# ShittyWizard/DiplomJourney

Measured on AMD Instinct MI355X. Metric: candidate N-step rollouts/sec + MPC-step p50 latency, 1/2/4/8 MI355X, higher is better.
Workload: dtype f64

## Files before the change

### diplomjourney_amd/csrc/mpc_episode.h

```cpp
#pragma once

#include <hip/hip_runtime.h>
#include <stddef.h>
#include <stdint.h>

#include "../../include/mpc_rollout.h"
#include "mpc_device.h"
#include "mpc_winner.h"

namespace mpc {

struct EpisodeHead {
  Consts K;
  double incumbent;
  double x, y, phi, v, beta;
  double x_t, y_t, x_0, y_0;
  double t;
  uint64_t seed;
  int64_t step;
  int32_t p, m, steps_for_slowing, episodes;
  int32_t nv, nb;
  int32_t recursive;
  int32_t has_traj;
};
// ... 26 lines not shown
constexpr int kStagedWords = kStoredWords + kEarlyWords;
static_assert(kStagedWords <= 64, "staged head: one word per lane");
constexpr int kLogWords = static_cast<int>(sizeof(mpc_episode_log_t) / 8);
static_assert(sizeof(EpisodeHead) % 8 == 0 && kHeadWords <= 64, "head: one word per lane");
static_assert(sizeof(mpc_episode_log_t) % 8 == 0 && kLogWords <= 64, "log: one word per lane");

__device__ __forceinline__ mpc_episode_log_t* log_slot(mpc_episode_log_t* log, int cap,
                                                       int64_t step) {
  return (log && cap > 0) ? &log[step % cap] : nullptr;
}

__device__ __forceinline__ bool early_pose_ok(const mpc_episode_config_t& c, const EpisodeHead& H,
                                              double x, double y) {
  if (c.stop_rule == 1 && x == H.x && y == H.y && H.recursive >= 1) return false;
  const double ex = H.x_t - x, ey = H.y_t - y;
  return !(ex * ex + ey * ey <= c.eps);
}

constexpr int kEpMaxGrid = 64;

constexpr int kConstsWords = static_cast<int>(sizeof(Consts) / 4);
constexpr int kPubWords = kConstsWords + 2;
static_assert(sizeof(Consts) % 4 == 0 && kPubWords <= 64, "published words: one wave");

struct EpisodeState {
  EpisodeHead h;
  StaleTraj st;
  EarlyPub early;
  double grid_v[kEpMaxGrid];
  double grid_b[kEpMaxGrid];
  uint32_t done;
  uint32_t chain_error;
  uint32_t p2p_seq;
  alignas(128) uint64_t chain_pub[kPubWords];
  alignas(128) uint64_t gathered_tag;
};
static_assert(offsetof(EpisodeState, st) == sizeof(EpisodeHead), "stale trajectory follows the head");
static_assert(offsetof(EpisodeState, early) == kStoredWords * 8, "EarlyPub follows the stale trajectory");

__device__ inline Consts episode_consts(const EpisodeHead& S, double x, double y, double phi,
                                        double L, double t_a, double t_b) {
  mpc_problem_t p;
  p.x = x;
  p.y = y;
  p.phi = phi;
  p.x_t = S.x_t;
  p.y_t = S.y_t;
  p.x_0 = S.x_0;
  p.y_0 = S.y_0;
  p.L = L;
  p.t_a = t_a;
  p.t_b = t_b;
  return consts_from_problem(p);
}

__device__ inline void episode_restart(const mpc_episode_config_t& c, EpisodeHead& S) {
  S.x = c.start_x;
  S.y = c.start_y;
  S.phi = c.start_phi;
// ... 40 lines not shown
                      !(c.max_steps > 0 && S.p + 1 > c.max_steps);
  const int k = S.m == 2 ? 2 : (S.m == 1 ? 1 : 0);
  E.k = common ? k : -1;
  E.x = S.has_traj ? st.ot[k][0] : S.x;
  E.y = S.has_traj ? st.ot[k][1] : S.y;
  E.ph = S.has_traj ? st.ot[k][2] : S.phi;
  E.alt = early_pose_ok(c, S, E.x, E.y) ? 1 : 0;
}

__global__ void k_episode_reset(mpc_episode_config_t c, EpisodeState* __restrict__ S) {
  if (threadIdx.x != 0) return;
  EpisodeHead H = {};
  episode_restart(c, H);
  episode_prepare(c, H);
  EarlyPub E;
  episode_early_prepare(c, H, S->st, E);
  S->early = E;
  S->h = H;
  S->done = 0u;
  S->chain_error = 0u;
  S->p2p_seq = 0u;
  for (int q = 0; q < kPubWords; ++q) S->chain_pub[q] = 0ull;
  S->gathered_tag = 0ull;
}

__device__ inline void turn_target(double ax, double ay, double aphi, double d, double R,
                                   double sign, double& tx, double& ty) {
  const double pi = 3.141592653589793;
  double sn, cs;
  if (pi / 2 <= aphi && aphi <= 3 * pi / 2) {
    if (aphi <= pi) {
      trig::sincos_fast(aphi - pi / 2, &sn, &cs);
      tx = ax - sign * d * cs - R * sn;
      ty = ay - sign * d * sn + R * cs;
    } else {
      trig::sincos_fast(aphi - pi, &sn, &cs);
      tx = ax + sign * d * sn - R * cs;
      ty = ay - sign * d * cs - R * sn;
    }
  } else if (aphi <= 2 * pi) {
    trig::sincos_fast(aphi - 3 * pi / 2, &sn, &cs);
    tx = ax + sign * d * cs + R * sn;
    ty = ay + sign * d * sn - R * cs;
  } else {
    trig::sincos_fast(aphi, &sn, &cs);
    tx = ax - sign * d * sn + R * cs;
// ... 137 lines not shown
```

### diplomjourney_amd/csrc/mpc_finalize.h

```cpp
#pragma once

#include <hip/hip_runtime.h>
#include <stddef.h>
#include <stdint.h>

#include <type_traits>

#include "../../include/mpc_rollout.h"
#include "mpc_argmin.h"
#include "mpc_device.h"
#include "mpc_episode.h"
#include "mpc_lanes.h"
#include "mpc_winner.h"

namespace mpc {

__device__ __forceinline__ void store_update(EpisodeHead* H, const uint64_t* s_head,
                                             mpc_episode_log_t* slot, const uint64_t* s_log,
                                             uint64_t* chain_pub, int chain_words,
                                             uint32_t epoch = 0, bool published = false,
                                             const uint32_t* pub = nullptr) {
  const int q = threadIdx.x;
  if (chain_pub && q < chain_words && !published) {
    if (epoch) {
// ... 39 lines not shown
  base = reinterpret_cast<const Rec*>(
      (static_cast<uint64_t>(static_cast<uint32_t>(__builtin_amdgcn_readfirstlane(
           static_cast<int>(ab >> 32)))) << 32) |
      static_cast<uint32_t>(__builtin_amdgcn_readfirstlane(static_cast<int>(ab))));
  asm volatile(
      "s_nop 4\n\t"
      "global_load_dwordx4 %0, %8, %16 sc1\n\t"
      "global_load_dwordx4 %1, %9, %16 sc1\n\t"
      "global_load_dwordx4 %2, %10, %16 sc1\n\t"
      "global_load_dwordx4 %3, %11, %16 sc1\n\t"
      "global_load_dwordx4 %4, %12, %16 sc1\n\t"
      "global_load_dwordx4 %5, %13, %16 sc1\n\t"
      "global_load_dwordx4 %6, %14, %16 sc1\n\t"
      "global_load_dwordx4 %7, %15, %16 sc1\n\t"
      "s_waitcnt vmcnt(0)"
      : "=&v"(r[0]), "=&v"(r[1]), "=&v"(r[2]), "=&v"(r[3]), "=&v"(r[4]), "=&v"(r[5]),
        "=&v"(r[6]), "=&v"(r[7])
      : "v"(o[0]), "v"(o[1]), "v"(o[2]), "v"(o[3]), "v"(o[4]), "v"(o[5]), "v"(o[6]), "v"(o[7]),
        "s"(base)
      : "memory");
}

struct NoRecSrc {};
template <int INTEG, int ROT, bool KDEV, int NT, bool SC1, bool GEN = false, bool TILED = false,
          class Src = NoRecSrc>
__device__ __forceinline__ void finalize_block(
    const Rec* __restrict__ part, int n_part, const Consts& K, const double* __restrict__ v,
    const double* __restrict__ b, int64_t n_cand, int n_steps, int64_t index_base,
    double incumbent, mpc_result_t* __restrict__ out, const mpc_episode_config_t& ecfg,
    const EpisodeHook& hook, EmitLds* lds, const Src& src = Src{}) {
  static_assert(NT >= 128, "head staging by wave 1");
  static_assert(MPC_MAX_STEPS * 3 <= NT, "trajectory stored one value per lane");
  __shared__ uint64_t s_head[kStagedWords];
  __shared__ mpc_episode_log_t s_log;
  __shared__ mpc_episode_log_t* s_slot;
  __shared__ uint64_t s_key[NT / 64];
  __shared__ int64_t s_idx[NT / 64];
  constexpr int kKWords = static_cast<int>(sizeof(Consts) / 4);
  __shared__ __attribute__((aligned(8))) uint32_t s_pub[64];
  __shared__ double2 s_sc[3];
  __shared__ int s_early, s_pose, s_sc_ready;
  uint64_t k = ~0ull;
  int64_t i = INT64_MAX;
  const bool stage = KDEV && hook.H && threadIdx.x >= 64 && threadIdx.x < 64 + kStagedWords;
  const uint64_t head_word =
      stage ? reinterpret_cast<const uint64_t*>(hook.H)[threadIdx.x - 64] : 0ull;
  if constexpr (!std::is_same_v<Src, NoRecSrc>) {
    src(k, i);
  } else if constexpr (SC1) {
    static_assert(kMaxBlocks <= 8 * NT, "load8_rec_sc1 covers 8 records per thread");
    const Rec* ptr[8];
    u64x2 r[8];
#pragma unroll
// ... 155 lines not shown
              if (pose == 1 && sc == 1) {
                Kp.s0 = s_sc[jj_w].x;
                Kp.c0 = s_sc[jj_w].y;
                pub = 1;
              }
            }
          }
          s_early = pub;
        }
        __builtin_amdgcn_fence(__ATOMIC_RELEASE, "wavefront");
        __builtin_amdgcn_wave_barrier();
        __builtin_amdgcn_fence(__ATOMIC_ACQUIRE, "wavefront");
        const int w3 = q - 192;
        if (s_early && w3 < hook.chain_pub_words)
          __hip_atomic_store(&hook.chain_pub[w3],
                             (static_cast<uint64_t>(s_pub[w3]) << 32) | hook.publish_epoch,
                             __ATOMIC_RELAXED, __HIP_MEMORY_SCOPE_AGENT);
      }
    };
    emit_winner<INTEG, ROT>(K, v, b, n_cand, n_steps, k, i, index_base + i, incumbent, out, lds,
                            &w, s_pv, s_pb, KDEV && hook.H, side_a, side_b, on_layer);
  }
  if (KDEV && hook.H) {
    const bool early = hook.publish_epoch && s_early;
    if (threadIdx.x == 0) {
      bool bad = false;
      episode_hook(ecfg, hook, w, *reinterpret_cast<EpisodeHead*>(s_head),
                   *reinterpret_cast<StaleTraj*>(&s_head[kHeadWords]), s_log, s_slot,
                   early ? s_pub : nullptr, &bad);
      if (bad && hook.chain_error) *hook.chain_error = 6u;
    }
    __syncthreads();
    if (hook.publish_epoch && threadIdx.x == 64) {
      EarlyPub E;
      episode_early_prepare(ecfg, *reinterpret_cast<const EpisodeHead*>(s_head),
                            *reinterpret_cast<const StaleTraj*>(&s_head[kHeadWords]), E);
      *reinterpret_cast<EarlyPub*>(reinterpret_cast<uint64_t*>(hook.H) + kStoredWords) = E;
    }
    store_update(hook.H, s_head, s_slot, reinterpret_cast<const uint64_t*>(&s_log),
                 hook.chain_pub, hook.chain_pub_words, hook.publish_epoch, early, s_pub);
    emit_winner_tail<INTEG, ROT>(K, n_steps, lds, out);
  }
}

template <int INTEG, int ROT>
__global__ __launch_bounds__(kFinBlock) void k_finalize_gen(
    const Rec* __restrict__ part, int n_part, const Consts* __restrict__ Kdev,
    const double* __restrict__ part_v, const double* __restrict__ part_b, int n_steps,
    int64_t index_base, const double* __restrict__ incumbent_dev,
    mpc_result_t* __restrict__ out, mpc_episode_config_t ecfg, EpisodeHook hook) {
  const Consts K = *Kdev;
  __shared__ EmitLds lds;
  finalize_block<INTEG, ROT, true, kFinBlock, false, true>(part, n_part, K, part_v, part_b, 0,
                                                           n_steps, index_base, *incumbent_dev,
                                                           out, ecfg, hook, &lds);
}

template <int INTEG, int ROT, bool KDEV, bool TILED = false>
__global__ __launch_bounds__(kFinBlock) void k_finalize(
    const Rec* __restrict__ part, int n_part, Consts Karg, const Consts* __restrict__ Kdev,
    const double* __restrict__ v, const double* __restrict__ b, int64_t n_cand, int n_steps,
    int64_t index_base, double incumbent_arg, const double* __restrict__ incumbent_dev,
    mpc_result_t* __restrict__ out, mpc_episode_config_t ecfg, EpisodeHook hook) {
  const Consts K = KDEV ? *Kdev : Karg;
// ... 54 lines not shown
```

### diplomjourney_amd/csrc/mpc_generated.h

```cpp
#pragma once

#include <hip/hip_runtime.h>
#include <stdint.h>

#include "mpc_argmin.h"
#include "mpc_device.h"
#include "mpc_episode.h"
#include "mpc_sampler.h"

namespace mpc {

__device__ inline void episode_grids(const mpc_episode_config_t& c, const EpisodeHead& S,
                                     double* s_v, double* s_b, int& nv_out, int& nb_out) {
  const int lane = threadIdx.x & 63;
  const uint64_t below = (lane == 0) ? 0ull : (~0ull >> (64 - lane));
  const int n_v = 1 + 2 * static_cast<int>(c.ratio_v);
  int nv = 0;
  double vmin = __builtin_inf();
  for (int base = 0; base < n_v; base += 64) {
    const int i = base + lane;
    const double cand = S.v + c.delta_v * (static_cast<double>(i) - c.ratio_v);
    const bool ok = i < n_v && !(cand < 0.0) && cand < c.v_max;
    const uint64_t m = __ballot(ok);
    const int pos = nv + __popcll(m & below);
    if (ok && pos < kEpMaxGrid) s_v[pos] = cand;
    if (S.steps_for_slowing > 0) {
      double mn = ok ? cand : __builtin_inf();
      for (int off = 32; off > 0; off >>= 1) mn = fmin(mn, __shfl_xor(mn, off, 64));
      vmin = fmin(vmin, mn);
    }
    nv += __popcll(m);
  }
  nv = nv < kEpMaxGrid ? nv : kEpMaxGrid;
  if (S.steps_for_slowing > 0 && nv > 0) {
    const double vel = vmin > c.v_min ? vmin : c.v_min;
// ... 177 lines not shown
```

### diplomjourney_amd/csrc/mpc_rollout.hip

```cpp
#include <hip/hip_ext.h>
#include <hip/hip_runtime.h>

#include <math.h>
#include <stdint.h>
#include <string.h>

#include <algorithm>
#include <mutex>
#include <type_traits>

#include "../../include/mpc_rollout.h"
#include "mpc_argmin.h"
#include "mpc_chain.h"
#include "mpc_comm.h"
#include "mpc_device.h"
#include "mpc_episode.h"
#include "mpc_episode_obs.h"
#include "mpc_episodes.h"
#include "mpc_exchange.h"
#include "mpc_finalize.h"
#include "mpc_ftepisodes.h"
#include "mpc_fulltree.h"
#include "mpc_generated.h"
#include "mpc_host_consts.h"
#include "mpc_kernels.h"
#include "mpc_lanes.h"
#include "mpc_run.h"
#include "mpc_sampler.h"
#include "mpc_winner.h"

namespace mpc {
namespace {

inline bool aligned16(const void* p) { return (reinterpret_cast<uintptr_t>(p) & 15u) == 0; }

inline int64_t cdiv(int64_t a, int64_t b) { return (a + b - 1) / b; }
// ... 652 lines not shown
            launched = hipFuncSetAttribute(
                           reinterpret_cast<const void*>(&k_rollout_generated<I, R, PL2>),
                           hipFuncAttributeMaxDynamicSharedMemorySize,
                           static_cast<int>(lds)) == hipSuccess;
          if (launched) {
            k_rollout_generated<I, R, PL2><<<grid, kBlock, lds, st>>>(
                *cfg, S, n_cand, n_steps, index_base, part, part_v, part_b);
            launched = hipPeekAtLastError() == hipSuccess;
          }
        },
        length_pow2(cfg->L));
    if (launched)
      k_finalize_gen<I, R><<<1, kFinBlock, 0, st>>>(part, static_cast<int>(grid), &S->h.K, part_v,
                                                    part_b, n_steps, index_base, &S->h.incumbent,
                                                    out, *cfg, hook);
  });
  if (!launched) {
    (void)hipGetLastError();
    return MPC_ERR_HIP;
  }
  return last_hip_status();
}

int mpc_episode_partials(void* state, const double* v_sc, const double* beta_sc, int64_t n_cand,
                         int32_t n_steps, int32_t integrator, void* ws, size_t ws_bytes,
                         mpc_stream_t stream) {
  if (check_episode_arrays(state, v_sc, beta_sc, n_cand, n_steps) != MPC_OK) return MPC_ERR_ARG;
  if (mode_ok(integrator) != MPC_OK) return MPC_ERR_UNSUPPORTED;
  if (!workspace_ok(ws, ws_bytes, n_cand, n_steps)) return MPC_ERR_WORKSPACE;
  EpisodeState* S = static_cast<EpisodeState*>(state);
  launch_rollout<true>(reinterpret_cast<hipStream_t>(stream), integrator, Consts{}, &S->h.K, v_sc,
                       beta_sc, n_cand, n_steps, static_cast<Rec*>(ws));
  return last_hip_status();
}

int mpc_episode_finalize(void* state, const double* v_sc, const double* beta_sc, int64_t n_cand,
                         int32_t n_steps, int64_t index_base, int32_t integrator, void* ws,
                         size_t ws_bytes, mpc_result_t* out, const mpc_episode_config_t* advance,
                         mpc_episode_log_t* log, int32_t log_capacity, mpc_stream_t stream) {
  const int a = check_episode_finish(state, v_sc, beta_sc, n_cand, n_steps, index_base, integrator,
                                     true, ws, ws_bytes, out, advance, log_capacity);
  if (a != MPC_OK) return a;
  EpisodeState* S = static_cast<EpisodeState*>(state);
  const int n_part = static_cast<int>(is_tiled(integrator)
                                          ? rollout_grid<kCplWide>(n_cand)
                                          : partial_count(v_sc, beta_sc, n_cand, false));
// ... 802 lines not shown
```

### diplomjourney_amd/device_episode.py

```python
import ctypes
import weakref

import torch

from . import native
from .abi import (CANDIDATE_BYTES, INTEGRATORS, IPC_HANDLE_BYTES, LOG_BYTES, MPC_LAYOUT_TILED,
                  MPC_MAX_OBSTACLES, MPC_TILE, RESULT_BYTES, MpcEpisodeLog, make_obstacles)
from .distributed import gather_bytes, gather_into, gather_results, reduce_int, shard_range
from .episode_config import ChainError, reference_episode_config
from .streams import _check_overlap_stream


def _is_tiled(controls):
    return isinstance(controls, torch.Tensor)


def _stop(events):
    if events:
        events[1].record()


class _ChainForm:
    pends_controls = False

# ... 4 lines not shown
class _OneGpuChain(_ChainForm):
    pends_controls = True

    def launch(self, ep, ctl, pend, events):
        vp, bp, integ = ep._ptrs(ctl)
        ws, ws_prev = ep._ws
        args = (1, ep._next_epoch(), vp, bp, *ep._shard, integ, ws.data_ptr(),
                ws_prev.data_ptr(), ws.numel(), *ep._prev_ptrs(pend), ep.local.data_ptr(), None, 0)
        if ep._n_obs or ep._obstacle_entries:
            log, cap, st = ep._tail()
            ep._C.mpc_episode_chain_step_obstacles(*ep._head, *ep._circles(), *args, log, cap,
                                                   ep._blocked_ptr(), st)
        else:
            ep._C.mpc_episode_chain_step(*ep._head, *args, *ep._tail())
        _stop(events)
        return ctl

    def flush(self, ep, pend):
        vp, bp, integ = ep._ptrs(pend)
        ws = ep._ws[1]
        ep._C.mpc_episode_finalize(
            ep.state.data_ptr(), vp, bp, *ep._shard, integ, ws.data_ptr(), ws.numel(),
            ep.local.data_ptr(), ctypes.byref(ep.cfg), *ep._tail())


class _P2PChain(_ChainForm):
    pends_controls = True

    def __init__(self, mailbox):
        self.mailbox = mailbox
        self.prev_epoch = 0

    def launch(self, ep, ctl, pend, events):
        vp, bp, integ = ep._ptrs(ctl)
        ws, ws_prev = ep._ws
        epoch = ep._next_epoch()
        ep._C.mpc_episode_p2p_step(
            *ep._head, epoch, self.prev_epoch if pend is not None else 0, vp, bp,
            *ep._shard, integ, ws.data_ptr(), ws_prev.data_ptr(), ws.numel(),
            *ep._prev_ptrs(pend), ctypes.c_void_p(self.mailbox.ptr), ep.world,
            ep.winner.data_ptr(), *ep._tail())
        _stop(events)
        self.prev_epoch = epoch
        return ctl

    def flush(self, ep, pend):
# ... 162 lines not shown
            raise ValueError(self._OBSTACLE_FORMS)
        self.cand = torch.zeros(CANDIDATE_BYTES, dtype=torch.uint8, device=dev)
        self.overlap = bool(overlap)
        if self.overlap and not (self.exchange and self.chain):
            raise ValueError("overlap: the chained exchange step only (exchange=True, chain=True)")
        if self.overlap and self.world > 32:
            raise ValueError("overlap: at most 32 ranks (gathered candidates staged in LDS)")
        self.p2p = bool(p2p)
        if self.p2p and (self.overlap or not (self.exchange and self.chain)):
            raise ValueError("p2p: the chained exchange step (exchange=True, chain=True), "
                             "not overlapped")
        self._mailbox = None
        self.p2p_status = None
        if self.p2p:
            self._p2p_setup(dev, bool(mailbox_uncached))
        self._form = (_OneGpuChain() if not self.exchange else
                      _P2PChain(self._mailbox) if self.p2p else
                      _OverlappedChain(self.world, dev) if self.overlap else _GatheredChain())
        if self.generate and self.exchange:
            raise ValueError("generated controls: one GPU (no exchange step)")
        self._gen_ws = None
        self._run_ws = None
        self._pending = None
        self._epoch = 0
        self._checked = {}
        self.steps_enqueued = 0
        self.n_blocked = torch.zeros(1, dtype=torch.int64, device=dev)
        self._obs, self._n_obs = None, 0
        self._obstacle_entries = False
        self._count_blocked = True
        self.set_obstacles(obstacles)
        self.reset(_fresh_mailbox=True)

    _OBSTACLE_FORMS = ("keep-out circles: the two-launch step (split=True, generate=False) and "
                       "the one-GPU chained step (chain=True, exchange=False) only")

    def set_obstacles(self, circles):
        obs, n = make_obstacles(circles)
        if n > MPC_MAX_OBSTACLES:
            raise ValueError(f"at most {MPC_MAX_OBSTACLES} obstacles")
        if n and not self._takes_obstacles():
            raise ValueError(self._OBSTACLE_FORMS)
        if self._pending is not None:
            self.flush()
        self._obs, self._n_obs = obs, n

# ... 95 lines not shown
        self._remember(key, v, b)
        return v, b

    def _check_tiled(self, t):
        key = (id(t), t.data_ptr())
        if self._seen(key, t):
            return t
        if (tuple(t.shape) != (-(-self.n_local // MPC_TILE), self.n_steps, 2, MPC_TILE)
                or t.dtype != torch.float64 or not t.is_contiguous()
                or t.device != self.v_sc.device or t.data_ptr() % 16):
            raise ValueError("tiled controls must be a contiguous 16-B aligned float64 "
                             "[ceil(n_local / 512), n_steps, 2, 512] tensor on the episode's "
                             "device (Expansion.sample_controls_tiled)")
        self._remember(key, t)
        return t

    def _chain_step(self, controls, events=None):
        form = self._form
        ctl = self._check_controls(controls)
        tiled = _is_tiled(ctl)
        if tiled and not form.pends_controls:
            raise ValueError("tiled controls: the one-GPU and P2P chained steps only")
        self.cur = ctl
        pend = self._pending
        if form.pends_controls and pend is not None and _is_tiled(pend) != tiled:
            raise ValueError("a chained episode keeps one control layout until its flush")
        if events:
            events[0].record()
        self._pending = form.launch(self, ctl, pend, events)
        if pend is not None:
            self.steps_enqueued += 1
        self._ws.reverse()

    def run(self, batches):
        if self.exchange:
            raise ValueError("the persistent run: one GPU (no exchange step)")
        if self._n_obs:
            raise ValueError("run(): " + self._OBSTACLE_FORMS)
        if self.integrator != "rect+cum" or self.n_local % 2:
            raise ValueError("the persistent run streams rect+cum candidates, n_local even")
        batches = list(batches)
        if not batches:
            return
        self.flush()
        ctls = [self._check_controls(c) for c in batches]
        tiled = _is_tiled(ctls[0])
        if any(_is_tiled(c) != tiled for c in ctls):
            raise ValueError("one control layout per run")
        if not tiled and any(not self._chainable(c) for c in ctls):
            raise ValueError("SoA controls of a run must be 16-B aligned")
        ptrs = [self._ptrs(c) for c in ctls]
        k = len(ptrs)
        V = (ctypes.c_void_p * k)(*[p[0] for p in ptrs])
        B = (ctypes.c_void_p * k)(*[p[1] for p in ptrs])
        if self._run_ws is None:
            self._run_ws = torch.zeros(self.lib.mpc_episode_run_workspace_bytes(self.n_local),
                                       dtype=torch.uint8, device=self.state.device)
        if self._epoch + k >= 0xFFFFFFF0:
            self._epoch = 0
        e0 = self._epoch + 1
        self._epoch += k
        self._C.mpc_episode_run(
            *self._head, e0, V, B, k, *self._shard, ptrs[0][2], self._run_ws.data_ptr(),
            self._run_ws.numel(), self.local.data_ptr(), *self._tail())
        self.cur = ctls[-1]
        self.steps_enqueued += k

    def _next_epoch(self):
        self._epoch = self._epoch % 0xFFFFFFFE + 1
        return self._epoch

    def flush(self):
        pend, self._pending = self._pending, None
        if pend is None:
            return
        self._form.flush(self, pend)
        self.steps_enqueued += 1

    def chain_error(self, local=False):
        e = ctypes.c_int32(0)
        self._C.mpc_episode_chain_error(self.state.data_ptr(), ctypes.byref(e),
                                        native.current_stream())
        return int(e.value) if local else self._all_ranks(e.value, "max")

    def _generate_step(self, events):
        if self._gen_ws is None:
            self._gen_ws = torch.empty(self.lib.mpc_episode_generate_workspace_bytes(
                self.n_local, self.n_steps), dtype=torch.uint8, device=self.state.device)
        if events:
            events[0].record()
        self._C.mpc_episode_generate_step(
            *self._head, *self._shard, self._integ, self._gen_ws.data_ptr(),
            self._gen_ws.numel(), self.local.data_ptr(), *self._tail())
        _stop(events)
        self.steps_enqueued += 1

    def expand(self, events=None, controls=None):
        C, st = self._C, native.current_stream()
        self.flush()
# ... 34 lines not shown
        v, b = self.cur
        st = st if st is not None else native.current_stream()
        if self._n_obs or self._obstacle_entries:
            self._C.mpc_episode_partials_obstacles(
                self.state.data_ptr(), *self._circles(), v.data_ptr(), b.data_ptr(), self.n_local,
                self.n_steps, self._integ, self.ws.data_ptr(), self.ws.numel(),
                self._blocked_ptr(), st)
            return
        self._C.mpc_episode_partials(
            self.state.data_ptr(), v.data_ptr(), b.data_ptr(), self.n_local,
            self.n_steps, self._integ, self.ws.data_ptr(), self.ws.numel(), st)

    def advance(self):
        if not self.exchange:
            return
        gathered = gather_results(self.local, self.group)
        self._C.mpc_episode_advance(*self._head, gathered.data_ptr(), self.world, *self._tail())
        self.steps_enqueued += 1

    def step(self, events=None, controls=None):
        if self.chain and controls is not None and self._chainable(controls):
            self._chain_step(controls, events)
            return
        if controls is not None and _is_tiled(controls):
            raise ValueError("tiled controls: chained rect+cum steps only (chain=True)")
        self.expand(events, controls)
        self.advance()

    def _chainable(self, controls):
        if self.integrator != "rect+cum" or self.n_local % 2:
            return False
        return _is_tiled(controls) or (controls[0].data_ptr() % 16 == 0
                                       and controls[1].data_ptr() % 16 == 0)

    def read_log(self):
        self.flush()
        torch.cuda.current_stream().synchronize()
        err = self.chain_error()
        if err:
            raise ChainError(err)
        if self._log_host is None:
            self._log_host = torch.empty(self.log.numel(), dtype=torch.uint8).pin_memory()
        self._log_host.copy_(self.log, non_blocking=True)
        torch.cuda.current_stream().synchronize()
        raw = self._log_host.numpy().tobytes()
        n = min(self.steps_enqueued, self.log_capacity)
# ... 6 lines not shown
```

### diplomjourney_amd/native.py

```python
import ctypes
import os
import subprocess
import sys
import types
from ctypes import POINTER, c_char_p, c_int, c_size_t, c_uint32, c_uint64

import torch

from .abi import MpcEpisodeConfig, MpcError, MpcFulltreeProblem, MpcProblem

PKG_DIR = os.path.dirname(os.path.abspath(__file__))
REPO_DIR = os.path.dirname(PKG_DIR)
LIB_NAME = "libmpc_rollout.so"
LIB_PATH = os.path.join(PKG_DIR, LIB_NAME)
SRC = os.path.join(PKG_DIR, "csrc", "mpc_rollout.hip")
HEADER = os.path.join(REPO_DIR, "include", "mpc_rollout.h")

_P = ctypes.c_void_p
_PP = POINTER(_P)
_I32 = ctypes.c_int32
_I64 = ctypes.c_int64
_D = ctypes.c_double
_PROB = POINTER(MpcProblem)
_CFG = POINTER(MpcEpisodeConfig)
# ... 34 lines not shown
    "mpc_episode_finalize": (c_int, _FINALIZE),
    "mpc_episode_step": (c_int, _FINALIZE),
    "mpc_episode_chain_step": (c_int, [_CFG, _P, _I32, c_uint32, _P, _P, _I64, _I32, _I64, _I32,
                                       _P, _P, c_size_t, _P, _P, _P, _P, _I32, _P, _I32, _P]),
    "mpc_episode_partials_obstacles": (c_int, [_P, _P, _I32, _P, _P, _I64, _I32, _I32, _P,
                                               c_size_t, _P, _P]),
    "mpc_episode_step_obstacles": (c_int, _FINALIZE[:1] + [_P, _I32] + _FINALIZE[1:-1] + [_P, _P]),
    "mpc_episode_chain_step_obstacles": (c_int, [_CFG, _P, _P, _I32, _I32, c_uint32, _P, _P, _I64,
                                                 _I32, _I64, _I32, _P, _P, c_size_t, _P, _P, _P,
                                                 _P, _I32, _P, _I32, _P, _P]),
    "mpc_episode_run_workspace_bytes": (c_size_t, [_I64]),
    "mpc_episode_run": (c_int, [_CFG, _P, c_uint32, _PP, _PP, _I32, _I64, _I32, _I64, _I32, _P,
                                c_size_t, _P, _P, _I32, _P]),
    "mpc_episode_exchange_step": (c_int, [_CFG, _P, c_uint32, _P, _P, _I64, _I32, _I64, _I32, _P,
                                          c_size_t, _P, _I32, _P, _P, _P, _I32, _P]),
    "mpc_episode_exchange_step2": (c_int, [_CFG, _P, c_uint32, c_uint32, _P, _P, _I64, _I32, _I64,
                                           _I32, _P, c_size_t, _P, _I32, _P, _P, _P, _I32, _P]),
    "mpc_episode_exchange_mark": (c_int, [_P, c_uint32, _P]),
    "mpc_episode_exchange_flush": (c_int, [_CFG, _P, _I32, _P, _I32, _P, _P, _I32, _P]),
    "mpc_episode_chain_error": (c_int, [_P, POINTER(_I32), _P]),
    "mpc_episode_generate_workspace_bytes": (c_size_t, [_I64, _I32]),
    "mpc_episode_generate_step": (c_int, [_CFG, _P, _I64, _I32, _I64, _I32, _P, c_size_t, _P, _P,
                                          _I32, _P]),
    "mpc_stream_create_cu_reserved": (c_int, [_I32, _PP]),
    "mpc_stream_create_cu_share": (c_int, [_I32, _I32, _PP]),
    "mpc_stream_destroy": (c_int, [_P]),
    "mpc_mailbox_bytes": (c_size_t, [_I32]),
    "mpc_mailbox_alloc": (c_int, [_I32, _I32, _PP]),
    "mpc_mailbox_free": (c_int, [_P]),
    "mpc_mailbox_set_peers": (c_int, [_P, _I32, _I32, _PP]),
    "mpc_mailbox_ping": (c_int, [_P, c_uint32, _P, _P]),
    "mpc_mailbox_clear": (c_int, [_P, _I32, _P]),
    "mpc_ipc_handle": (c_int, [_P, _P]),
    "mpc_ipc_open": (c_int, [_P, _PP]),
    "mpc_ipc_close": (c_int, [_P]),
    "mpc_peer_enable": (c_int, [_I32]),
    "mpc_episode_p2p_step": (c_int, [_CFG, _P, c_uint32, c_uint32, _P, _P, _I64, _I32, _I64, _I32,
                                     _P, _P, c_size_t, _P, _P, _P, _I32, _P, _P, _I32, _P]),
    "mpc_episode_p2p_flush": (c_int, [_CFG, _P, c_uint32, _P, _P, _I64, _I32, _I64, _I32, _P,
                                      c_size_t, _P, _I32, _P, _P, _I32, _P]),
    "mpc_comm_unique_id": (c_int, [_P]),
    "mpc_comm_init_rank": (c_int, [_P, _I32, _I32, _PP]),
    "mpc_comm_init_all": (c_int, [_I32, POINTER(_I32), _PP]),
    "mpc_comm_destroy": (c_int, [_P]),
    "mpc_exchange_allgather": (c_int, [_P, _P, _P, _P]),
    "mpc_exchange_allgather_group": (c_int, [_I32, _PP, _PP, _PP, _PP]),
# ... 107 lines not shown
```

### include/mpc_rollout.h

```cpp
#ifndef DIPLOMJOURNEY_AMD_MPC_ROLLOUT_H
#define DIPLOMJOURNEY_AMD_MPC_ROLLOUT_H

#include <stddef.h>
#include <stdint.h>

#ifdef __cplusplus
extern "C" {
#endif

typedef struct ihipStream_t* mpc_stream_t;

#define MPC_MAX_STEPS 32

enum {
  MPC_OK = 0,
  MPC_ERR_ARG = -1,
  MPC_ERR_WORKSPACE = -2,
  MPC_ERR_HIP = -3,
  MPC_ERR_UNSUPPORTED = -4
};

enum { MPC_INTEG_QK21 = 0, MPC_INTEG_RECT = 1 };

#define MPC_HEADING_ROTATE 0x100
// ... 230 lines not shown
int mpc_episode_p2p_flush(const mpc_episode_config_t* cfg, void* state, uint32_t last_epoch,
                          const double* v_last, const double* beta_last, int64_t n_cand,
                          int32_t n_steps, int64_t index_base, int32_t integrator,
                          const void* ws_last, size_t ws_bytes, void* mailbox, int32_t world,
                          mpc_result_t* out, mpc_episode_log_t* log, int32_t log_capacity,
                          mpc_stream_t stream);

typedef struct mpc_comm* mpc_comm_t;
int mpc_comm_unique_id(void* id );
int mpc_comm_init_rank(const void* id, int32_t n_ranks, int32_t rank, mpc_comm_t* comm);
int mpc_comm_init_all(int32_t n_devices, const int32_t* devices, mpc_comm_t* comms);
int mpc_comm_destroy(mpc_comm_t comm);
int mpc_exchange_allgather(mpc_comm_t comm, const mpc_candidate_t* local,
                           mpc_candidate_t* gathered, mpc_stream_t stream);
int mpc_exchange_allgather_group(int32_t n, const mpc_comm_t* comms,
                                 const mpc_candidate_t* const* local,
                                 mpc_candidate_t* const* gathered, const mpc_stream_t* streams);

size_t mpc_episode_generate_workspace_bytes(int64_t n_cand, int32_t n_steps);
int mpc_episode_generate_step(const mpc_episode_config_t* cfg, void* state, int64_t n_cand,
                              int32_t n_steps, int64_t index_base, int32_t integrator, void* ws,
                              size_t ws_bytes, mpc_result_t* out, mpc_episode_log_t* log,
                              int32_t log_capacity, mpc_stream_t stream);
int mpc_episode_chain_error(const void* state, int32_t* error, mpc_stream_t stream);

typedef struct mpc_episodes_progress {
  int32_t calls;
  int32_t stop;
  int64_t candidates;
} mpc_episodes_progress_t;
size_t mpc_episodes_state_bytes(int32_t n_robots);
int mpc_episodes_reset(const mpc_episode_config_t* cfgs, int32_t n_robots, void* state,
                       mpc_stream_t stream);
int mpc_episodes_run(void* state, int32_t n_robots, int32_t n_steps, int32_t integrator,
                     int32_t max_calls, mpc_episode_log_t* log, int32_t log_capacity,
                     mpc_episodes_progress_t* progress, mpc_stream_t stream);

typedef struct mpc_fulltree_problem {
  double x, y, phi;
  double x_t, y_t, x_0, y_0;
  double atan_target;
  double L, t_a, t_b;
} mpc_fulltree_problem_t;

typedef struct mpc_fulltree_result {
  double cost;
// ... 46 lines not shown
```

Before: 33.98 billion.

## Chain generated-control episode steps in one kernel with speculative draw precompute

Adds a chained kernel for generated-control episode steps. Block 0 finalizes the previous step's winner and publishes the next step's velocity, beta, seed and grid size through an epoch-tagged mailbox. The other blocks read those published words, speculatively precompute random grid draws, then roll out candidate pairs from an LDS grid table. This removes a separate finalize launch and the host round trip between steps, at the cost of spin-waiting on device flags, a speculative seed path that is discarded when it misses, and more complex flush handling in Python.

```diff
diff --git a/diplomjourney_amd/csrc/mpc_chain_gen.h b/diplomjourney_amd/csrc/mpc_chain_gen.h
--- /dev/null
+++ b/diplomjourney_amd/csrc/mpc_chain_gen.h
@@ -0,0 +1,313 @@
+#pragma once
+
+#include <hip/hip_runtime.h>
+#include <stddef.h>
+#include <stdint.h>
+
+#include "../../include/mpc_rollout.h"
+#include "mpc_argmin.h"
+#include "mpc_chain.h"
+#include "mpc_device.h"
+#include "mpc_episode.h"
+#include "mpc_exchange.h"
+#include "mpc_finalize.h"
+#include "mpc_generated.h"
+#include "mpc_sampler.h"
+#include "mpc_winner.h"
+
+namespace mpc {
+
+
+constexpr int kGpV = 0, kGpBeta = 2, kGpSlow = 4, kGpSeed = 5, kGpGrid = 7;
+static_assert(kGpGrid + 1 == kGenPubWords, "gen_pub layout");
+constexpr int kGenAllWords = kPubWords + kGenPubWords;
+static_assert(kGenAllWords <= 64, "published words: one wave");
+
+__device__ __forceinline__ void gen_publish(EpisodeState* S, uint32_t epoch, double v, double beta,
+                                            int32_t slow, uint64_t seed, uint32_t n_grid) {
+  const int q = threadIdx.x;
+  if (q >= kGenPubWords) return;
+  const uint64_t vb = static_cast<uint64_t>(__double_as_longlong(v));
+  const uint64_t bb = static_cast<uint64_t>(__double_as_longlong(beta));
+  const uint64_t two = q < kGpBeta ? vb : q < kGpSlow ? bb : seed;
+  uint32_t d;
+  if (q == kGpSlow)
+    d = static_cast<uint32_t>(slow);
+  else if (q == kGpGrid)
+    d = n_grid;
+  else
+    d = static_cast<uint32_t>(((q - (q < kGpSlow ? 0 : kGpSeed)) & 1) ? two >> 32 : two);
+  __hip_atomic_store(&S->gen_pub[q], (static_cast<uint64_t>(d) << 32) | epoch, __ATOMIC_RELAXED,
+                     __HIP_MEMORY_SCOPE_AGENT);
+}
+
+__device__ __forceinline__ void gen_open_step(const mpc_episode_config_t& c, EpisodeState* S,
+                                              EpisodeHead& H, uint32_t epoch, double* s_v,
+                                              double* s_b) {
+  __shared__ int s_n[2];
+  if (threadIdx.x < 64) {
+    int nv, nb;
+    episode_grids(c, H, s_v, s_b, nv, nb);
+    if (threadIdx.x == 0) {
+      s_n[0] = nv;
+      s_n[1] = nb;
+      H.nv = nv;
+      H.nb = nb;
+    }
+  }
+  __syncthreads();
+  const int nv = s_n[0], nb = s_n[1], q = threadIdx.x;
+  if (q < nv)
+    S->grid_v[q] = s_v[q];
+  else if (q >= 64 && q - 64 < nb)
+    S->grid_b[q - 64] = s_b[q - 64];
+  gen_publish(S, epoch, H.v, H.beta, H.steps_for_slowing, H.seed,
+              static_cast<uint32_t>(nv) * static_cast<uint32_t>(nb));
+}
+
+struct GenNext {
+  const mpc_episode_config_t* c;
+  EpisodeState* S;
+  uint32_t epoch;
+  double *s_v, *s_b;
+  __device__ __forceinline__ void operator()(uint64_t* s_head) const {
+    gen_open_step(*c, S, *reinterpret_cast<EpisodeHead*>(s_head), epoch, s_v, s_b);
+  }
+};
+
+__device__ __forceinline__ void gen_read(const EpisodeState* S, uint32_t* s_w, uint32_t* s_tag) {
+  const int q = threadIdx.x;
+  if (q < kGenAllWords) {
+    const uint64_t* p = q < kPubWords ? &S->chain_pub[q] : &S->gen_pub[q - kPubWords];
+    const uint64_t w = __hip_atomic_load(const_cast<uint64_t*>(p), __ATOMIC_RELAXED,
+                                         __HIP_MEMORY_SCOPE_AGENT);
+    s_w[q] = static_cast<uint32_t>(w >> 32);
+    s_tag[q] = static_cast<uint32_t>(w);
+  }
+}
+
+__device__ __forceinline__ uint32_t gen_word(const uint32_t* s_w, int i) {
+  return static_cast<uint32_t>(__builtin_amdgcn_readfirstlane(s_w[kPubWords + i]));
+}
+__device__ __forceinline__ uint64_t gen_word2(const uint32_t* s_w, int i) {
+  return (static_cast<uint64_t>(gen_word(s_w, i + 1)) << 32) | gen_word(s_w, i);
+}
+
+__device__ __forceinline__ void gen_draws(uint32_t* s_idx, uint64_t seed, uint32_t n_grid,
+                                          uint64_t g0, int n_steps) {
+  static_assert(kEpMaxGrid * kEpMaxGrid <= (1 << 16), "a grid index fits 16 bits");
+#pragma unroll 4
+  for (int st = 0; st < n_steps; ++st) {
+    const uint32_t i0 = grid_entry(seed, st, g0, n_grid, 1);
+    const uint32_t i1 = grid_entry(seed, st, g0 + 1, n_grid, 1);
+    s_idx[st * kBlock + threadIdx.x] = i0 | (i1 << 16);
+  }
+}
+
+template <int INTEG, int ROT, bool PL2>
+__device__ __forceinline__ void drawn_lane(const Consts& K, const double2* s_grid,
+                                           const uint32_t* idx, int n_steps, double (&cst)[2]) {
+  double x[2], y[2], ph[2], sn[2], cs[2];
+  bool bad[2];
+#pragma unroll
+  for (int j = 0; j < 2; ++j) {
+    step_start<ROT>(K, x[j], y[j], ph[j], sn[j], cs[j]);
+    bad[j] = false;
+  }
+  trig::Leads lead = trig::const_leads();
+#pragma unroll 1
+  for (int st = 0; st < n_steps; ++st) {
+    const uint32_t d = idx[st * kBlock];
+    const double2 e0 = s_grid[d & 0xffffu];
+    const double2 e1 = s_grid[d >> 16];
+    double ph0 = ROT ? 0.0 : ph[0], ph1 = ROT ? 0.0 : ph[1];
+    step_core<INTEG, ROT, PL2>(x[0], y[0], ph0, sn[0], cs[0], e0.x, e0.y, K, bad[0], &lead);
+    step_core<INTEG, ROT, PL2>(x[1], y[1], ph1, sn[1], cs[1], e1.x, e1.y, K, bad[1], &lead);
+    if (!ROT) {
+      ph[0] = ph0;
+      ph[1] = ph1;
+    }
+  }
+  if constexpr (ROT == kRotCum) {
+#pragma unroll
+    for (int j = 0; j < 2; ++j)
+      if (!bad[j]) cum_pose<PL2>(K, x[j], y[j], x[j], y[j]);
+  }
+#pragma unroll
+  for (int j = 0; j < 2; ++j) {
+    if (bad[j]) {
+      x[j] = K.x;
+      y[j] = K.y;
+      ph[j] = K.phi;
+      for (int sr = 0; sr < n_steps; ++sr) {
+        const uint32_t d = idx[sr * kBlock];
+        const double2 e = s_grid[j ? d >> 16 : d & 0xffffu];
+        step_safe<INTEG>(x[j], y[j], ph[j], e.x, e.y, K);
+      }
+    }
+    cst[j] = cost(x[j], y[j], K);
+  }
+}
+
+template <int INTEG, int ROT, bool PL2>
+__device__ __forceinline__ void gen_tiles(const mpc_episode_config_t& c,
+                                          EpisodeState* __restrict__ S, uint32_t epoch,
+                                          int64_t n_cand, int n_steps, int64_t base,
+                                          Rec* __restrict__ part, double* __restrict__ part_v,
+                                          double* __restrict__ part_b, int has_prev,
+                                          double2* s_grid, uint32_t* s_idx, double* s_v,
+                                          double* s_b) {
+  __shared__ __attribute__((aligned(16))) uint32_t s_w[64];
+  __shared__ uint32_t s_tag[64];
+  __shared__ int s_mode, s_nv, s_nb;
+  const int64_t n_tiles = (n_cand + kBlock * 2 - 1) / (kBlock * 2);
+  const int64_t tile0 = static_cast<int64_t>(blockIdx.x) - 1;
+  if (threadIdx.x < 64) {
+    gen_read(S, s_w, s_tag);
+    const int q = threadIdx.x;
+    const uint32_t tag = q < kGenAllWords ? s_tag[q] : epoch;
+    const bool fin = __ballot(tag != epoch) == 0;
+    const bool spec_w = q >= kPubWords + kGpSeed && q < kGenAllWords;
+    const bool spec = has_prev && __ballot(spec_w && tag != epoch - 1u) == 0;
+    if (q == 0) s_mode = fin ? 2 : spec ? 1 : 0;
+  }
+  __syncthreads();
+  const int mode = __builtin_amdgcn_readfirstlane(s_mode);
+  uint64_t seed_s = 0;
+  uint32_t ng_s = 0;
+  const int64_t c_first = tile0 * (kBlock * 2) + threadIdx.x * 2;
+  if (mode) {
+    seed_s = gen_word2(s_w, kGpSeed) + (mode == 1 ? 0x9E3779B9ull : 0ull);
+    ng_s = gen_word(s_w, kGpGrid);
+    if (tile0 < n_tiles && c_first < n_cand)
+      gen_draws(s_idx, seed_s, ng_s, static_cast<uint64_t>(base + c_first), n_steps);
+  }
+  if (mode != 2) {
+    __syncthreads();
+    if (threadIdx.x < 64) {
+      const int q = threadIdx.x;
+      const uint64_t* const pw = q < kPubWords ? &S->chain_pub[q]
+                                 : &S->gen_pub[q < kGenAllWords ? q - kPubWords : 0];
+      auto ld = [&]() {
+        return __hip_atomic_load(const_cast<uint64_t*>(pw), __ATOMIC_RELAXED,
+                                 __HIP_MEMORY_SCOPE_AGENT);
+      };
+      auto here = [&](uint64_t w) {
+        return __ballot(q < kGenAllWords && static_cast<uint32_t>(w) != epoch) == 0;
+      };
+      const uint32_t deadline = wall_deadline(kChainWaitTicks);
+      bool fin = false;
+      uint64_t a = ld(), b = 0, got = 0;
+      for (;;) {
+        __builtin_amdgcn_s_sleep(2);
+        b = ld();
+        if (here(a)) { got = a; fin = true; break; }
+        if (wall_passed(deadline)) break;
+        __builtin_amdgcn_s_sleep(2);
+        a = ld();
+        if (here(b)) { got = b; fin = true; break; }
+        if (wall_passed(deadline)) break;
+      }
+      if (q < kGenAllWords) s_w[q] = static_cast<uint32_t>((fin ? got : a) >> 32);
+      if (!fin && q == 0) S->chain_error = 1u;
+    }
+    __syncthreads();
+  }
+  if (threadIdx.x < 64) {
+    const double v = __longlong_as_double(static_cast<long long>(gen_word2(s_w, kGpV)));
+    const double beta = __longlong_as_double(static_cast<long long>(gen_word2(s_w, kGpBeta)));
+    int nv, nb;
+    const GridSrc src{v, beta, static_cast<int32_t>(gen_word(s_w, kGpSlow))};
+    episode_grids(c, src, s_v, s_b, nv, nb);
+    if (threadIdx.x == 0) {
+      s_nv = nv;
+      s_nb = nb;
+    }
+  }
+  __syncthreads();
+  const int nv = s_nv, nb = s_nb;
+  const uint32_t n_grid = static_cast<uint32_t>(nv) * static_cast<uint32_t>(nb);
+  for (uint32_t k = threadIdx.x; k < n_grid; k += kBlock)
+    s_grid[k] = make_double2(s_v[k / nb], s_b[k % nb]);
+  const uint64_t seed = gen_word2(s_w, kGpSeed);
+  bool drawn = mode != 0 && seed == seed_s && n_grid == ng_s;
+  const Consts K = consts_from_words(s_w);
+  __syncthreads();
+  uint64_t best_k = ~0ull;
+  int64_t best_i = INT64_MAX;
+  if (n_grid > 0) {
+    for (int64_t tile = tile0; tile < n_tiles; tile += gridDim.x - 1) {
+      const int64_t c0 = tile * (kBlock * 2) + threadIdx.x * 2;
+      if (c0 < n_cand) {
+        if (!drawn) gen_draws(s_idx, seed, n_grid, static_cast<uint64_t>(base + c0), n_steps);
+        double cst[2];
+        drawn_lane<INTEG, ROT, PL2>(K, s_grid, s_idx + threadIdx.x, n_steps, cst);
+#pragma unroll
+        for (int j = 0; j < 2; ++j) {
+          const uint64_t kk = cost_key_nonneg(cst[j]);
+          if (kk < best_k) {
+            best_k = kk;
+            best_i = c0 + j;
+          }
+        }
+      }
+      drawn = false;
+    }
+  }
+  block_argmin(best_k, best_i);
+  if (threadIdx.x == 0) part[blockIdx.x - 1] = Rec{best_k, best_i};
+  __shared__ int64_t s_best;
+  if (threadIdx.x == 0) s_best = best_k == ~0ull ? -1 : best_i;
+  __syncthreads();
+  const int64_t bi = s_best;
+  if (bi >= 0 && threadIdx.x < n_steps) {
+    const double2 e =
+        s_grid[grid_entry(seed, threadIdx.x, static_cast<uint64_t>(base + bi), n_grid, 1)];
+    part_v[(blockIdx.x - 1) * MPC_MAX_STEPS + threadIdx.x] = e.x;
+    part_b[(blockIdx.x - 1) * MPC_MAX_STEPS + threadIdx.x] = e.y;
+  }
+}
+
+#ifndef MPC_CHAIN_GEN_WAVES
+#define MPC_CHAIN_GEN_WAVES 5
+#endif
+
+__host__ __device__ inline size_t chain_gen_lds(int64_t grid_entries, int n_steps) {
+  const size_t n = static_cast<size_t>(grid_entries) * sizeof(double2) +
+                   static_cast<size_t>(n_steps) * kBlock * sizeof(uint32_t);
+  return n > sizeof(EmitLds) ? n : sizeof(EmitLds);
+}
+
+template <int INTEG, int ROT, bool PL2>
+__global__ __launch_bounds__(kBlock, MPC_CHAIN_GEN_WAVES) void k_episode_chain_gen(
+    mpc_episode_config_t c, EpisodeState* __restrict__ S, uint32_t epoch, int64_t n_cand,
+    int n_steps, int64_t base, int grid_entries, Rec* __restrict__ part,
+    double* __restrict__ part_v, double* __restrict__ part_b, int has_prev,
+    const Rec* __restrict__ part_prev, const double* __restrict__ pv_prev,
+    const double* __restrict__ pb_prev, mpc_result_t* __restrict__ out_prev,
+    mpc_episode_log_t* __restrict__ log, int cap) {
+  static_assert(ROT == kRotCum, "chained steps need the pose-independent recurrence");
+  extern __shared__ double2 s_chain_gen[];
+  __shared__ double s_v[kEpMaxGrid], s_b[kEpMaxGrid];
+  if (blockIdx.x == 0) {
+    if (has_prev) {
+      const Consts Kp = S->h.K;
+      const EpisodeHook hook{&S->h, log, cap, S->chain_pub, kPubWords, epoch, &S->chain_error};
+      finalize_block<INTEG, ROT, true, kBlock, false, true, false>(
+          part_prev, static_cast<int>(gridDim.x) - 1, Kp, pv_prev, pb_prev, 0, n_steps, base,
+          S->h.incumbent, out_prev, c, hook, reinterpret_cast<EmitLds*>(s_chain_gen), NoRecSrc{},
+          GenNext{&c, S, epoch, s_v, s_b});
+    } else {
+      gen_open_step(c, S, S->h, epoch, s_v, s_b);
+      chain_publish(S, epoch);
+    }
+    __syncthreads();
+    if (threadIdx.x == 0 && (S->h.K.L_pow2 != 0) != PL2) S->chain_error = 2u;
+    return;
+  }
+  gen_tiles<INTEG, ROT, PL2>(c, S, epoch, n_cand, n_steps, base, part, part_v, part_b, has_prev,
+                             s_chain_gen,
+                             reinterpret_cast<uint32_t*>(s_chain_gen + grid_entries), s_v, s_b);
+}
+
+}
diff --git a/diplomjourney_amd/csrc/mpc_episode.h b/diplomjourney_amd/csrc/mpc_episode.h
--- a/diplomjourney_amd/csrc/mpc_episode.h
+++ b/diplomjourney_amd/csrc/mpc_episode.h
@@ -72,6 +72,7 @@
 constexpr int kConstsWords = static_cast<int>(sizeof(Consts) / 4);
 constexpr int kPubWords = kConstsWords + 2;
 static_assert(sizeof(Consts) % 4 == 0 && kPubWords <= 64, "published words: one wave");
+constexpr int kGenPubWords = 8;
 
 struct EpisodeState {
   EpisodeHead h;
@@ -84,7 +85,11 @@
   uint32_t p2p_seq;
   alignas(128) uint64_t chain_pub[kPubWords];
   alignas(128) uint64_t gathered_tag;
-};
+  uint64_t gen_pub[kGenPubWords];
+};
+static_assert(offsetof(EpisodeState, gen_pub) + kGenPubWords * 8 <=
+                  offsetof(EpisodeState, gathered_tag) + 128,
+              "gen_pub fits in gathered_tag's line");
 static_assert(offsetof(EpisodeState, st) == sizeof(EpisodeHead), "stale trajectory follows the head");
 static_assert(offsetof(EpisodeState, early) == kStoredWords * 8, "EarlyPub follows the stale trajectory");
 
@@ -171,6 +176,7 @@
   S->p2p_seq = 0u;
   for (int q = 0; q < kPubWords; ++q) S->chain_pub[q] = 0ull;
   S->gathered_tag = 0ull;
+  for (int q = 0; q < kGenPubWords; ++q) S->gen_pub[q] = 0ull;
 }
 
 __device__ inline void turn_target(double ax, double ay, double aphi, double d, double R,
diff --git a/diplomjourney_amd/csrc/mpc_finalize.h b/diplomjourney_amd/csrc/mpc_finalize.h
--- a/diplomjourney_amd/csrc/mpc_finalize.h
+++ b/diplomjourney_amd/csrc/mpc_finalize.h
@@ -85,13 +85,14 @@
 }
 
 struct NoRecSrc {};
+struct NoNext {};
 template <int INTEG, int ROT, bool KDEV, int NT, bool SC1, bool GEN = false, bool TILED = false,
-          class Src = NoRecSrc>
+          class Src = NoRecSrc, class Next = NoNext>
 __device__ __forceinline__ void finalize_block(
     const Rec* __restrict__ part, int n_part, const Consts& K, const double* __restrict__ v,
     const double* __restrict__ b, int64_t n_cand, int n_steps, int64_t index_base,
     double incumbent, mpc_result_t* __restrict__ out, const mpc_episode_config_t& ecfg,
-    const EpisodeHook& hook, EmitLds* lds, const Src& src = Src{}) {
+    const EpisodeHook& hook, EmitLds* lds, const Src& src = Src{}, const Next& next = Next{}) {
   static_assert(NT >= 128, "head staging by wave 1");
   static_assert(MPC_MAX_STEPS * 3 <= NT, "trajectory stored one value per lane");
   __shared__ uint64_t s_head[kStagedWords];
@@ -293,7 +294,7 @@
                             &w, s_pv, s_pb, KDEV && hook.H, side_a, side_b, on_layer);
   }
   if (KDEV && hook.H) {
-    const bool early = hook.publish_epoch && s_early;
+    const bool early = !GEN && hook.publish_epoch && s_early;
     if (threadIdx.x == 0) {
       bool bad = false;
       episode_hook(ecfg, hook, w, *reinterpret_cast<EpisodeHead*>(s_head),
@@ -302,7 +303,8 @@
       if (bad && hook.chain_error) *hook.chain_error = 6u;
     }
     __syncthreads();
-    if (hook.publish_epoch && threadIdx.x == 64) {
+    if constexpr (GEN && !std::is_same_v<Next, NoNext>) next(s_head);
+    if (!GEN && hook.publish_epoch && threadIdx.x == 64) {
       EarlyPub E;
       episode_early_prepare(ecfg, *reinterpret_cast<const EpisodeHead*>(s_head),
                             *reinterpret_cast<const StaleTraj*>(&s_head[kHeadWords]), E);
@@ -311,6 +313,10 @@
     store_update(hook.H, s_head, s_slot, reinterpret_cast<const uint64_t*>(&s_log),
                  hook.chain_pub, hook.chain_pub_words, hook.publish_epoch, early, s_pub);
     emit_winner_tail<INTEG, ROT>(K, n_steps, lds, out);
+    if constexpr (GEN) {
+      if (!hook.publish_epoch && hook.chain_pub && threadIdx.x < kGenPubWords)
+        reinterpret_cast<EpisodeState*>(hook.H)->gen_pub[threadIdx.x] = 0ull;
+    }
   }
 }
 
diff --git a/diplomjourney_amd/csrc/mpc_generated.h b/diplomjourney_amd/csrc/mpc_generated.h
--- a/diplomjourney_amd/csrc/mpc_generated.h
+++ b/diplomjourney_amd/csrc/mpc_generated.h
@@ -10,7 +10,12 @@
 
 namespace mpc {
 
-__device__ inline void episode_grids(const mpc_episode_config_t& c, const EpisodeHead& S,
+struct GridSrc {
+  double v, beta;
+  int32_t steps_for_slowing;
+};
+template <class Head>
+__device__ inline void episode_grids(const mpc_episode_config_t& c, const Head& S,
                                      double* s_v, double* s_b, int& nv_out, int& nb_out) {
   const int lane = threadIdx.x & 63;
   const uint64_t below = (lane == 0) ? 0ull : (~0ull >> (64 - lane));
diff --git a/diplomjourney_amd/csrc/mpc_rollout.hip b/diplomjourney_amd/csrc/mpc_rollout.hip
--- a/diplomjourney_amd/csrc/mpc_rollout.hip
+++ b/diplomjourney_amd/csrc/mpc_rollout.hip
@@ -12,6 +12,7 @@
 #include "../../include/mpc_rollout.h"
 #include "mpc_argmin.h"
 #include "mpc_chain.h"
+#include "mpc_chain_gen.h"
 #include "mpc_comm.h"
 #include "mpc_device.h"
 #include "mpc_episode.h"
@@ -710,6 +711,90 @@
   return last_hip_status();
 }
 
+static int check_generate(const mpc_episode_config_t* cfg, const void* state, int64_t n_cand,
+                          int32_t n_steps, int64_t index_base, int32_t integrator, const void* ws,
+                          size_t ws_bytes, int32_t log_capacity, bool chained) {
+  if (check_episode_cfg(cfg) != MPC_OK || !state || n_steps < 1 || n_steps > MPC_MAX_STEPS ||
+      index_base < 0 || log_capacity < 0)
+    return MPC_ERR_ARG;
+  if (n_cand < 2 || n_cand % 2 != 0) return MPC_ERR_ARG;
+  if (mode_ok(integrator) != MPC_OK || cfg->enumerate) return MPC_ERR_UNSUPPORTED;
+  if (chained && !chained_mode_ok(integrator, false)) return MPC_ERR_UNSUPPORTED;
+  if (!ws || ws_bytes < mpc_episode_generate_workspace_bytes(n_cand, n_steps))
+    return MPC_ERR_WORKSPACE;
+  return MPC_OK;
+}
+
+int mpc_episode_generate_chain_step(const mpc_episode_config_t* cfg, void* state, uint32_t epoch,
+                                    int64_t n_cand, int32_t n_steps, int64_t index_base,
+                                    int32_t integrator, void* ws, const void* ws_prev,
+                                    size_t ws_bytes, mpc_result_t* out_prev,
+                                    mpc_episode_log_t* log, int32_t log_capacity,
+                                    mpc_stream_t stream) {
+  if (epoch == 0) return MPC_ERR_ARG;
+  const int a = check_generate(cfg, state, n_cand, n_steps, index_base, integrator, ws, ws_bytes,
+                               log_capacity, true);
+  if (a != MPC_OK) return a;
+  if (ws_prev && (!out_prev || ws_prev == ws)) return MPC_ERR_ARG;
+  if (!wall_clock_ok()) return MPC_ERR_UNSUPPORTED;
+  const int64_t nv = std::min<int64_t>(kEpMaxGrid, 1 + 2 * static_cast<int64_t>(cfg->ratio_v));
+  const int64_t nb =
+      std::min<int64_t>(kEpMaxGrid, 1 + 2 * static_cast<int64_t>(cfg->ratio_beta));
+  const size_t lds = chain_gen_lds(nv * nb, n_steps);
+  EpisodeState* S = static_cast<EpisodeState*>(state);
+  hipStream_t st = reinterpret_cast<hipStream_t>(stream);
+  const int64_t tiles = gen_grid(n_cand);
+  auto ctl = [&](const void* w) {
+    return reinterpret_cast<double*>(static_cast<char*>(const_cast<void*>(w)) +
+                                     gen_ctl_offset(n_cand));
+  };
+  double* part_v = ctl(ws);
+  const double* pv_prev = ws_prev ? ctl(ws_prev) : nullptr;
+  bool launched = true;
+  dispatch_bools(
+      [&](auto PL2) {
+        auto* kern = &k_episode_chain_gen<MPC_INTEG_RECT, kRotCum, PL2>;
+        if (lds > 48 * 1024)
+          launched = hipFuncSetAttribute(reinterpret_cast<const void*>(kern),
+                                         hipFuncAttributeMaxDynamicSharedMemorySize,
+                                         static_cast<int>(lds)) == hipSuccess;
+        if (launched)
+          kern<<<tiles + 1, kBlock, lds, st>>>(
+              *cfg, S, epoch, n_cand, n_steps, index_base, static_cast<int>(nv * nb),
+              static_cast<Rec*>(ws), part_v, part_v + tiles * MPC_MAX_STEPS, ws_prev ? 1 : 0,
+              static_cast<const Rec*>(ws_prev), pv_prev,
+              pv_prev ? pv_prev + tiles * MPC_MAX_STEPS : nullptr, out_prev, log, log_capacity);
+      },
+      length_pow2(cfg->L));
+  if (!launched) {
+    (void)hipGetLastError();
+    return MPC_ERR_HIP;
+  }
+  return last_hip_status();
+}
+
+int mpc_episode_generate_finalize(const mpc_episode_config_t* cfg, void* state, int64_t n_cand,
+                                  int32_t n_steps, int64_t index_base, int32_t integrator,
+                                  const void* ws, size_t ws_bytes, mpc_result_t* out,
+                                  mpc_episode_log_t* log, int32_t log_capacity,
+                                  mpc_stream_t stream) {
+  if (!out) return MPC_ERR_ARG;
+  const int a = check_generate(cfg, state, n_cand, n_steps, index_base, integrator, ws, ws_bytes,
+                               log_capacity, false);
+  if (a != MPC_OK) return a;
+  EpisodeState* S = static_cast<EpisodeState*>(state);
+  const char* w = static_cast<const char*>(ws);
+  const int64_t grid = gen_grid(n_cand);
+  const double* part_v = reinterpret_cast<const double*>(w + gen_ctl_offset(n_cand));
+  const EpisodeHook hook = episode_hook(S, true, log, log_capacity);
+  dispatch_mode(integrator, [&](auto I, auto R) {
+    k_finalize_gen<I, R><<<1, kFinBlock, 0, reinterpret_cast<hipStream_t>(stream)>>>(
+        reinterpret_cast<const Rec*>(w), static_cast<int>(grid), &S->h.K, part_v,
+        part_v + grid * MPC_MAX_STEPS, n_steps, index_base, &S->h.incumbent, out, *cfg, hook);
+  });
+  return last_hip_status();
+}
+
 int mpc_episode_partials(void* state, const double* v_sc, const double* beta_sc, int64_t n_cand,
                          int32_t n_steps, int32_t integrator, void* ws, size_t ws_bytes,
                          mpc_stream_t stream) {
diff --git a/diplomjourney_amd/device_episode.py b/diplomjourney_amd/device_episode.py
--- a/diplomjourney_amd/device_episode.py
+++ b/diplomjourney_amd/device_episode.py
@@ -50,6 +50,30 @@
         ep._C.mpc_episode_finalize(
             ep.state.data_ptr(), vp, bp, *ep._shard, integ, ws.data_ptr(), ws.numel(),
             ep.local.data_ptr(), ctypes.byref(ep.cfg), *ep._tail())
+
+
+class _GeneratedChain(_ChainForm):
+
+    def __init__(self):
+        self._ws = None
+
+    def launch(self, ep, ctl, pend, events):
+        if self._ws is None:
+            n = ep.lib.mpc_episode_generate_workspace_bytes(ep.n_local, ep.n_steps)
+            self._ws = [torch.empty(n, dtype=torch.uint8, device=ep.state.device)
+                        for _ in range(2)]
+        ws = self._ws[1] if pend is self._ws[0] else self._ws[0]
+        ep._C.mpc_episode_generate_chain_step(
+            *ep._head, ep._next_epoch(), *ep._shard, ep._integ, ws.data_ptr(),
+            pend.data_ptr() if pend is not None else None, ws.numel(), ep.local.data_ptr(),
+            *ep._tail())
+        _stop(events)
+        return ws
+
+    def flush(self, ep, pend):
+        ep._C.mpc_episode_generate_finalize(
+            *ep._head, *ep._shard, ep._integ, pend.data_ptr(), pend.numel(), ep.local.data_ptr(),
+            *ep._tail())
 
 
 class _P2PChain(_ChainForm):
@@ -258,6 +282,8 @@
         self._gen_ws = None
         self._run_ws = None
         self._pending = None
+        self._pending_form = None
+        self._gen_form = _GeneratedChain()
         self._epoch = 0
         self._checked = {}
         self.steps_enqueued = 0
@@ -399,15 +425,33 @@
         if tiled and not form.pends_controls:
             raise ValueError("tiled controls: the one-GPU and P2P chained steps only")
         self.cur = ctl
+        if self._pending is not None and self._pending_form is not form:
+            self.flush()
         pend = self._pending
         if form.pends_controls and pend is not None and _is_tiled(pend) != tiled:
             raise ValueError("a chained episode keeps one control layout until its flush")
         if events:
             events[0].record()
         self._pending = form.launch(self, ctl, pend, events)
+        self._pending_form = form
         if pend is not None:
             self.steps_enqueued += 1
         self._ws.reverse()
+
+    def _gen_chainable(self):
+        return (self.generate and self.chain and not self.exchange and not self._n_obs
+                and not self._obstacle_entries and self.integrator == "rect+cum"
+                and self.n_local % 2 == 0 and not self.cfg.enumerate)
+
+    def _gen_chain_step(self, events=None):
+        form = self._gen_form
+        if events:
+            events[0].record()
+        pend = self._pending
+        self._pending = form.launch(self, None, pend, events)
+        self._pending_form = form
+        if pend is not None:
+            self.steps_enqueued += 1
 
     def run(self, batches):
         if self.exchange:
@@ -451,7 +495,7 @@
         pend, self._pending = self._pending, None
         if pend is None:
             return
-        self._form.flush(self, pend)
+        (self._pending_form or self._form).flush(self, pend)
         self.steps_enqueued += 1
 
     def chain_error(self, local=False):
@@ -532,6 +576,11 @@
         if self.chain and controls is not None and self._chainable(controls):
             self._chain_step(controls, events)
             return
+        if controls is None and self._gen_chainable():
+            if self._pending is not None and self._pending_form is not self._gen_form:
+                self.flush()
+            self._gen_chain_step(events)
+            return
         if controls is not None and _is_tiled(controls):
             raise ValueError("tiled controls: chained rect+cum steps only (chain=True)")
         self.expand(events, controls)
diff --git a/diplomjourney_amd/native.py b/diplomjourney_amd/native.py
--- a/diplomjourney_amd/native.py
+++ b/diplomjourney_amd/native.py
@@ -80,6 +80,10 @@
     "mpc_episode_generate_workspace_bytes": (c_size_t, [_I64, _I32]),
     "mpc_episode_generate_step": (c_int, [_CFG, _P, _I64, _I32, _I64, _I32, _P, c_size_t, _P, _P,
                                           _I32, _P]),
+    "mpc_episode_generate_chain_step": (c_int, [_CFG, _P, c_uint32, _I64, _I32, _I64, _I32, _P, _P,
+                                                c_size_t, _P, _P, _I32, _P]),
+    "mpc_episode_generate_finalize": (c_int, [_CFG, _P, _I64, _I32, _I64, _I32, _P, c_size_t, _P,
+                                              _P, _I32, _P]),
     "mpc_stream_create_cu_reserved": (c_int, [_I32, _PP]),
     "mpc_stream_create_cu_share": (c_int, [_I32, _I32, _PP]),
     "mpc_stream_destroy": (c_int, [_P]),
diff --git a/include/mpc_rollout.h b/include/mpc_rollout.h
--- a/include/mpc_rollout.h
+++ b/include/mpc_rollout.h
@@ -276,6 +276,17 @@
                               int32_t n_steps, int64_t index_base, int32_t integrator, void* ws,
                               size_t ws_bytes, mpc_result_t* out, mpc_episode_log_t* log,
                               int32_t log_capacity, mpc_stream_t stream);
+int mpc_episode_generate_chain_step(const mpc_episode_config_t* cfg, void* state, uint32_t epoch,
+                                    int64_t n_cand, int32_t n_steps, int64_t index_base,
+                                    int32_t integrator, void* ws, const void* ws_prev,
+                                    size_t ws_bytes, mpc_result_t* out_prev,
+                                    mpc_episode_log_t* log, int32_t log_capacity,
+                                    mpc_stream_t stream);
+int mpc_episode_generate_finalize(const mpc_episode_config_t* cfg, void* state, int64_t n_cand,
+                                  int32_t n_steps, int64_t index_base, int32_t integrator,
+                                  const void* ws, size_t ws_bytes, mpc_result_t* out,
+                                  mpc_episode_log_t* log, int32_t log_capacity,
+                                  mpc_stream_t stream);
 int mpc_episode_chain_error(const void* state, int32_t* error, mpc_stream_t stream);
 
 typedef struct mpc_episodes_progress {
```

Result: no change. 33.90 billion (-0.2%).
